# lambdaclass/simpleworks

Hardware: AMD Instinct MI355X
Metric: Marlin prove() constraints/sec at 2^20 R1CS; G1 MSM points/sec (higher is better)
Workload: dtype u32 limbs (384-bit Montgomery Fq for G1, 256-bit Fr); 1 GPU; marlin_prove: synthetic R1CS, 2^20 constraints = variables = non-zeros per matrix (|H| = |K| = 2^20), SRS + proving key device resident; per_gpu_units=1048576, multi_gpu=replicas (one proof per rank)

## Files before the change

### simpleworks_amd/_lib.py

```python
import ctypes
import json
import os

import numpy as np

_HERE = os.path.dirname(os.path.abspath(__file__))
LIB_PATH = os.environ.get("SWM_LIB_PATH") or os.path.join(_HERE, "libswmarlin.so")

_u64p = ctypes.POINTER(ctypes.c_uint64)
_u32p = ctypes.POINTER(ctypes.c_uint32)
_vp = ctypes.c_void_p
_sz = ctypes.c_size_t
_int = ctypes.c_int

ABI = {
    "swm_version": (_int, []),
    "swm_strerror": (ctypes.c_char_p, [_int]),
    "swm_init": (_int, [_int, ctypes.POINTER(_vp)]),
    "swm_destroy": (None, [_vp]),
    "swm_last_error": (ctypes.c_char_p, [_vp]),
    "swm_set_stream": (_int, [_vp, _vp]),
    "swm_set_msm_sharding": (_int, [_vp, ctypes.c_uint, ctypes.c_uint, _vp, _vp]),
    "swm_rccl_unique_id": (_int, [ctypes.c_void_p]),
    "swm_rccl_init": (_int, [_vp, ctypes.c_void_p, ctypes.c_uint, ctypes.c_uint]),
# ... 971 lines not shown
                                              _p64(out), _p64(jac) if backmap else None, _p32(status), n), "swm_selftest_p28")
        return out, status[:n], jac

    def _poly(self, op, data, n, m, z, pieces, out):
        zz = np.ascontiguousarray(z if z is not None else np.zeros(4), dtype=np.uint64).reshape(4)
        pc = np.ascontiguousarray(pieces if pieces is not None else np.zeros(2), dtype=np.uint64).reshape(-1)
        self._check(self.lib.swm_selftest_poly(self.h, op, data.ctypes.data, n, m, _p64(zz), _p64(pc), pc.size // 2,
                                               out.ctypes.data if out is not None else None), "swm_selftest_poly")

    def selftest_suffix_recurrence(self, a_mont, m, z_mont):
        a = np.ascontiguousarray(a_mont, dtype=np.uint64).reshape(-1, 4).copy()
        self._poly(0, a, a.shape[0], m, z_mont, None, None)
        return a

    def selftest_div_linear(self, p_mont, z_mont):
        p = np.ascontiguousarray(p_mont, dtype=np.uint64).reshape(-1, 4)
        out = np.zeros_like(p)
        self._poly(1, p, p.shape[0], 0, z_mont, None, out)
        return out

    def selftest_poly_eval(self, p_mont, z_mont):
        p = np.ascontiguousarray(p_mont, dtype=np.uint64).reshape(-1, 4)
        out = np.zeros(4, dtype=np.uint64)
        self._poly(2, p, p.shape[0], 0, z_mont, None, out)
        return out

    def selftest_poly_eval_many(self, buf_mont, pieces, z_mont):
        buf = np.ascontiguousarray(buf_mont, dtype=np.uint64).reshape(-1, 4)
        pc = np.asarray(pieces, dtype=np.uint64).reshape(-1, 2)
        out = np.zeros((pc.shape[0], 4), dtype=np.uint64)
        self._poly(3, buf, buf.shape[0], 0, z_mont, pc, out)
        return out

    def selftest_ntt_from(self, src_mont, log_n, inverse=False, coset=False):
        src = np.ascontiguousarray(src_mont, dtype=np.uint64).reshape(-1, 4).copy()
        out = np.zeros((1 << log_n, 4), dtype=np.uint64)
        self._poly(4 + int(bool(inverse)) + 2 * int(bool(coset)), src, src.shape[0], log_n, None, None, out)
        return out, src

    def selftest_ntt_cosets(self, coeffs_mont, log_n, ks):
        src = np.ascontiguousarray(coeffs_mont, dtype=np.uint64).reshape(-1, 4).copy()
        kk = np.ascontiguousarray(ks, dtype=np.uint64).reshape(-1)
        out = np.zeros((kk.size << log_n, 4), dtype=np.uint64)
        self._check(self.lib.swm_selftest_poly(self.h, 9, src.ctypes.data, src.shape[0], log_n, _p64(np.zeros(4, np.uint64)),
                                               _p64(kk), kk.size, out.ctypes.data), "swm_selftest_poly")
        return out.reshape(kk.size, 1 << log_n, 4)

    def selftest_intt_cosets3(self, evals_mont, log_n):
        ev = np.ascontiguousarray(evals_mont, dtype=np.uint64).reshape(-1, 4).copy()
        out = np.zeros_like(ev)
        self._poly(10, ev, ev.shape[0], log_n, None, None, out)
        return out

    def selftest_scan(self, words):
        w = np.ascontiguousarray(words, dtype=np.uint32).reshape(-1)
        out = np.zeros(w.size + 1, dtype=np.uint32)
        self._poly(8, w, w.size, 0, None, None, out)
        return out[:-1], int(out[-1])

    def selftest_sample_fr(self, rng, need):
        out = np.zeros((max(need, 1), 4), dtype=np.uint64)
        self._check(self.lib.swm_selftest_sample_fr(self.h, rng.h, need, _p64(out)), "swm_selftest_sample_fr")
        return out[:need]

    def selftest_mul_throughput(self, which, threads, iters):
        ms = ctypes.c_float(0)
        self._check(self.lib.swm_selftest_mul_throughput(self.h, which, threads, iters, ctypes.byref(ms)),
                    "swm_selftest_mul_throughput")
        return ms.value
```

### simpleworks_amd/csrc/fr29.cuh

```cuda
#pragma once
#include "ff.cuh"

namespace swm {

struct Fr29 {
    uint32_t l[9];
};
static constexpr uint32_t M29 = (1u << 29) - 1;
struct Fr29Consts {
    static constexpr uint32_t P[9] = SWM_FR29_P;
    static constexpr uint32_t ONE[9] = SWM_FR29_ONE;
    static constexpr uint32_t P2[9] = SWM_FR29_2P;
};

__device__ __forceinline__ Fr29 fr29_unpack(const Fr& a) {
    Fr29 r;
#pragma unroll
    for (int i = 0; i < 9; i++) {
        const int bit = 29 * i, w = bit >> 5, off = bit & 31;
        uint32_t v = a.v[w] >> off;
        if (off > 3 && w + 1 < 8) v |= a.v[w + 1] << (32 - off);
        r.l[i] = i < 8 ? (v & M29) : v;
    }
    return r;
}
__device__ __forceinline__ Fr fr29_pack(const Fr29& a) {
    Fr r;
#pragma unroll
    for (int w = 0; w < 8; w++) {
        const int bit = 32 * w, i = bit / 29, off = bit - 29 * i;
        uint32_t v = a.l[i] >> off;
        if (i + 1 < 9) v |= a.l[i + 1] << (29 - off);
        if (29 - off + 29 < 32 && i + 2 < 9) v |= a.l[i + 2] << (58 - off);
        r.v[w] = v;
    }
    return r;
}
__device__ __forceinline__ Fr29 fr29_const(const uint32_t (&c)[9]) {
    Fr29 r;
#pragma unroll
    for (int i = 0; i < 9; i++) r.l[i] = c[i];
    return r;
}
__device__ __forceinline__ Fr29 fr29_normalize(const Fr29& a) {
    Fr29 r;
    uint32_t c = 0;
#pragma unroll
    for (int i = 0; i < 8; i++) {
        uint32_t t = a.l[i] + c;
        r.l[i] = t & M29;
        c = t >> 29;
    }
    r.l[8] = a.l[8] + c;
    return r;
}
__device__ __forceinline__ Fr29 fr29_add(const Fr29& a, const Fr29& b) {
    Fr29 r;
#pragma unroll
    for (int i = 0; i < 9; i++) r.l[i] = a.l[i] + b.l[i];
    return r;
}
struct Spread29 {
    uint32_t l[9];
};
__device__ __forceinline__ Fr29 fr29_sub(const Fr29& a, const Fr29& b, const Spread29& sp) {
    Fr29 r;
#pragma unroll
    for (int i = 0; i < 9; i++) r.l[i] = a.l[i] + sp.l[i] - b.l[i];
    return r;
}
__device__ __forceinline__ Fr29 fr29_mul(const Fr29& a, const Fr29& b) {
    Fr29 r;
    uint32_t m[9];
    uint64_t acc = 0;
#pragma unroll
    for (int k = 0; k < 9; k++) {
#pragma unroll
        for (int i = 0; i <= k; i++) acc += (uint64_t)a.l[i] * b.l[k - i];
#pragma unroll
        for (int i = 0; i < k; i++) acc += (uint64_t)m[i] * Fr29Consts::P[k - i];
        m[k] = (0u - (uint32_t)acc) & M29;
        acc = (acc + m[k]) >> 29;
    }
#pragma unroll
    for (int k = 9; k < 17; k++) {
#pragma unroll
        for (int i = k - 8; i < 9; i++) acc += (uint64_t)a.l[i] * b.l[k - i];
#pragma unroll
        for (int i = k - 8; i < 9; i++) acc += (uint64_t)m[i] * Fr29Consts::P[k - i];
        r.l[k - 9] = (uint32_t)acc & M29;
        acc >>= 29;
    }
    r.l[8] = (uint32_t)acc;
    return r;
}
#include "fr29_mul_asm.inc"
__device__ __forceinline__ Fr29 fr29_mul_fenced(const Fr29& a, const Fr29& b) {
    Fr29 r;
    uint32_t m0, m1, m2, m3, m4, m5, m6, m7, m8;
    constexpr const uint32_t (&P)[9] = Fr29Consts::P;
    static_assert(P[0] == 1u, "the carry rule needs r = 1 mod 2^29");
    asm(SWM_FR29_MUL_ASM_TEXT
        : "=&v"(r.l[0]), "=&v"(r.l[1]), "=&v"(r.l[2]), "=&v"(r.l[3]), "=&v"(r.l[4]), "=&v"(r.l[5]), "=&v"(r.l[6]), "=&v"(r.l[7]),
          "=&v"(r.l[8]), "=&v"(m0), "=&v"(m1), "=&v"(m2), "=&v"(m3), "=&v"(m4), "=&v"(m5), "=&v"(m6), "=&v"(m7), "=&v"(m8)
        : "v"(a.l[0]), "v"(a.l[1]), "v"(a.l[2]), "v"(a.l[3]), "v"(a.l[4]), "v"(a.l[5]), "v"(a.l[6]), "v"(a.l[7]), "v"(a.l[8]),
          "v"(b.l[0]), "v"(b.l[1]), "v"(b.l[2]), "v"(b.l[3]), "v"(b.l[4]), "v"(b.l[5]), "v"(b.l[6]), "v"(b.l[7]), "v"(b.l[8]),
          "s"(P[1]), "s"(P[2]), "s"(P[3]), "s"(P[4]), "s"(P[5]), "s"(P[6]), "s"(P[7]), "s"(P[8]), "s"(M29), "s"((uint64_t)M29)
        : "v0", "v1", "vcc");
    return r;
}
__device__ __forceinline__ Fr29 fr29_cond_sub(const Fr29& a, const uint32_t (&k)[9]) {
    Fr29 t;
    uint32_t borrow = 0;
#pragma unroll
    for (int i = 0; i < 9; i++) {
        uint32_t d = a.l[i] - k[i] - borrow;
        borrow = d >> 31;
        t.l[i] = i < 8 ? (d & M29) : d;
    }
    Fr29 r;
#pragma unroll
// ... 10 lines not shown
```

### simpleworks_amd/csrc/marlin.hip

```cpp
#include <stdlib.h>
#include <string.h>
#include <algorithm>
#include <chrono>
#include <functional>
#include <memory>
#include <type_traits>
#include "devops.cuh"
#include "g1.cuh"
#include "host/ahp.h"

#include "msm.h"
using namespace swm;

#define LAUNCHX(ctx, name, kernel, grid, block, shmem, ...)                         \
    do {                                                                            \
        prof_begin(ctx, name);                                                      \
        hipLaunchKernelGGL(kernel, grid, block, shmem, (ctx)->stream, __VA_ARGS__); \
        prof_end(ctx);                                                              \
        hip_check(ctx, hipGetLastError(), name);                                    \
    } while (0)

#include "host/pk_codec.h"
#include "host/host_handles.h"
struct swm_srs {
// ... 2330 lines not shown
    SWM_ON_DEVICE(ctx);
    SWM_GUARD(ctx, *out = pk_deserialize(ctx, bytes, len, (flags & SWM_KEY_UNCOMPRESSED) != 0, !(flags & SWM_KEY_UNCHECKED)));
}
int swm_pk_deserialize(swm_ctx* ctx, const uint8_t* bytes, size_t len, swm_pk** out) {
    return swm_pk_deserialize_ex(ctx, bytes, len, 0, out);
}
int swm_r1cs_is_satisfied(swm_ctx* ctx, const swm_r1cs* cs, int* ok, size_t* first_bad) {
    if (!ctx || !cs || !ok) return SWM_ERR_INVALID_ARG;
    SWM_ON_DEVICE(ctx);
    SWM_GUARD(ctx, is_satisfied_impl(ctx, cs, ok, first_bad));
}

static void selftest_poly_impl(swm_ctx* ctx, int op, void* data, size_t n, size_t m, const uint64_t* z, const uint64_t* pieces,
                               size_t npieces, void* out) {
    Fr zz = fp_zero<Fr>();
    if (z) memcpy(zz.v, z, 32);
    if (op == 8) {
        DBuf<uint32_t> in(ctx, n), res(ctx, n);
        if (n) in.upload((const uint32_t*)data, n);
        const uint32_t total = scan_exclusive_u32(ctx, in.p, res.p, n);
        std::vector<uint32_t> h = res.download(0, n);
        if (n) memcpy(out, h.data(), n * 4);
        ((uint32_t*)out)[n] = total;
        return;
    }
    DVec a(ctx, n);
    if (n) a.upload((const Fr*)data, n);
    if (op == 9) {
        unsigned ks[4];
        for (size_t c = 0; c < npieces; c++) ks[c] = (unsigned)pieces[c];
        DVec t(ctx, npieces << m);
        rc_check(ctx, ntt_cosets_fwd(ctx, a.p, n, (unsigned)m, ks, (unsigned)npieces, t.p));
        std::vector<Fr> h = t.download(0, t.n);
        memcpy(out, h.data(), t.n * sizeof(Fr));
        return;
    }
    if (op == 10) {
        const size_t N = (size_t)1 << m;
        rc_check(ctx, ntt_cosets_inv(ctx, a.p, (unsigned)m, 3));
        DVec t(ctx, 3 * N);
        const Fr* u = a.p;
        Fr* o = t.p;
        const Fr iota = HDomain(4).gen, half = fr_half();
        ew(ctx, "cosets3_solve", N, [=] __device__(size_t j) {
            const Cosets3 c = cosets3_solve(u[j], u[j + N], u[j + 2 * N], iota, half);
            o[j] = c.p0;
            o[j + N] = c.p1;
            o[j + 2 * N] = c.p2;
        });
        std::vector<Fr> h = t.download(0, t.n);
        memcpy(out, h.data(), t.n * sizeof(Fr));
        return;
    }
    if (op == 0) {
        suffix_recurrence(ctx, a.p, n, m, zz);
        std::vector<Fr> h = a.download(0, n);
        if (n) memcpy(data, h.data(), n * sizeof(Fr));
    } else if (op == 1) {
        DivResult r = div_linear(ctx, a.p, n, zz);
        std::vector<Fr> h = r.work.download(0, n);
        if (n) memcpy(out, h.data(), n * sizeof(Fr));
    } else if (op == 2) {
        const Fr v = poly_eval(ctx, a.p, n, zz);
        memcpy(out, v.v, sizeof(Fr));
    } else if (op == 3) {
        for (size_t i = 0; i < npieces; i++)
            if (pieces[2 * i] > n || pieces[2 * i + 1] > n - pieces[2 * i]) throw MarlinError(SWM_ERR_INVALID_ARG, "piece out of range");
        DVec res(ctx, npieces);
        std::vector<EvalItem> items;
        for (size_t i = 0; i < npieces; i++) items.push_back({a.p + pieces[2 * i], (size_t)pieces[2 * i + 1], res.p + i});
        EvalPoint ep = eval_point(ctx, zz);
        poly_eval_many(ctx, items, ep);
        std::vector<Fr> h = res.download(0, npieces);
        if (npieces) memcpy(out, h.data(), npieces * sizeof(Fr));
    } else {
        DVec t = dv_ntt_from(ctx, a.p, n, (unsigned)m, ((op - 4) & 1) != 0, ((op - 4) & 2) != 0);
        std::vector<Fr> h = t.download(0, t.n);
        memcpy(out, h.data(), t.n * sizeof(Fr));
        std::vector<Fr> s = a.download(0, n);
        if (n) memcpy(data, s.data(), n * sizeof(Fr));
    }
}
int swm_selftest_poly(swm_ctx* ctx, int op, void* data, size_t n, size_t m, const uint64_t z[4], const uint64_t* pieces,
                      size_t npieces, void* out) {
    if (!ctx || op < 0 || op > 10 || (n && !data)) return SWM_ERR_INVALID_ARG;
    if ((op >= 1 && op <= 3 && !z) || (op == 0 && (!z || m == 0)) || (op != 0 && !out) || (op == 3 && npieces && !pieces))
        return SWM_ERR_INVALID_ARG;
    if (op >= 4 && op <= 7 && (m < 1 || m > 28 || n > ((size_t)1 << m))) return SWM_ERR_INVALID_ARG;
    if (op == 9) {
        if (m < 1 || m > 26 || n > ((size_t)2 << m) || npieces < 1 || npieces > 4 || !pieces) return SWM_ERR_INVALID_ARG;
        for (size_t c = 0; c < npieces; c++)
            if (pieces[c] > 3) return SWM_ERR_INVALID_ARG;
    }
    if (op == 10 && (m < 1 || m > 26 || n != ((size_t)3 << m))) return SWM_ERR_INVALID_ARG;
    SWM_ON_DEVICE(ctx);
    SWM_GUARD(ctx, selftest_poly_impl(ctx, op, data, n, m, z, pieces, npieces, out));
}
static void selftest_sample_impl(swm_ctx* ctx, ChaChaRng& rng, size_t need, uint64_t* out_mont) {
    DVec d(ctx, need);
    sample_fr_bulk(ctx, rng, d.p, need);
    std::vector<Fr> h = d.download(0, need);
    if (need) memcpy(out_mont, h.data(), need * sizeof(Fr));
}
int swm_selftest_sample_fr(swm_ctx* ctx, swm_rng* rng, size_t need, uint64_t* out_mont) {
    if (!ctx || !rng || (need && !out_mont)) return SWM_ERR_INVALID_ARG;
    SWM_ON_DEVICE(ctx);
    SWM_GUARD(ctx, selftest_sample_impl(ctx, rng->r, need, out_mont));
}

static void selftest_g1_codec_impl(swm_ctx* ctx, int op, const void* in, size_t n, void* out, unsigned* bad) {
    const dim3 grid((unsigned)((n + 255) / 256)), block(256);
    if (op == 0) {
        DBuf<G1Affine> pts(ctx, n);
        DBuf<uint32_t> enc(ctx, n * 24);
        pts.upload((const G1Affine*)in, n);
        LAUNCHX(ctx, "g1_encode_uncompressed", g1_encode_uncompressed_kernel, grid, block, 0, pts.p, n, enc.p);
        std::vector<uint32_t> h = enc.download(0, n * 24);
        memcpy(out, h.data(), n * 96);
        return;
    }
    DBuf<uint32_t> enc(ctx, n * 24), flag(ctx, 1);
    DBuf<G1Affine> pts(ctx, n);
    flag.zero();
    enc.upload((const uint32_t*)in, n * 24);
    if (op == 1) LAUNCHX(ctx, "g1_decode_uncompressed", g1_decode_uncompressed_kernel<true>, grid, block, 0, enc.p, n, pts.p, flag.p);
    else LAUNCHX(ctx, "g1_decode_unchecked", g1_decode_uncompressed_kernel<false>, grid, block, 0, enc.p, n, pts.p, flag.p);
    *bad = flag.download(0, 1)[0];
    std::vector<G1Affine> h = pts.download(0, n);
    memcpy(out, h.data(), n * sizeof(G1Affine));
}
int swm_selftest_g1_codec(swm_ctx* ctx, int op, const void* in, size_t n, void* out, unsigned* bad) {
    if (!ctx || op < 0 || op > 2 || (n && (!in || !out)) || (op != 0 && !bad) || n > ((size_t)1 << 31)) return SWM_ERR_INVALID_ARG;
    SWM_ON_DEVICE(ctx);
    if (op != 0) *bad = 0;
    if (n == 0) return SWM_OK;
    SWM_GUARD(ctx, selftest_g1_codec_impl(ctx, op, in, n, out, bad));
}

// ... 41 lines not shown
```

### simpleworks_amd/csrc/ntt.hip

```cpp
#include <atomic>
#include "context.h"
#include "ff.cuh"
#include "fr29.cuh"
#include <string.h>
#include <algorithm>
#include <vector>

namespace swm {

static constexpr int NTT_THREADS = 256;
static constexpr unsigned NTT_MAX_LOG_R = 10;

struct NttPassArgs {
    const Fr* src;
    Fr* dst;
    unsigned log_n, log_r, log_ns;
    const Fr* tw_small;
    const Fr* tw_lo;
    const Fr* tw_hi;
    const Fr* cs_lo;
    const Fr* cs_hi;
    uint64_t src_len;
    const Fr* pass_tw;
    int coset_in;
// ... 73 lines not shown
    for (; h >= 2; h >>= 2) {
        const unsigned hh = h >> 1, s1 = (R >> 1) / h, s2 = 2 * s1;
        for (unsigned q = threadIdx.x; q < (R >> 2) * J; q += NTT_THREADS) {
            unsigned jj = q % J, qq = q / J;
            unsigned p = qq & (hh - 1), blk = qq / hh;
            unsigned i0 = blk * 2 * h + p, i1 = i0 + hh, i2 = i0 + h, i3 = i2 + hh;
            Fr x0 = tile[i0 * J + jj], x1 = tile[i1 * J + jj], x2 = tile[i2 * J + jj], x3 = tile[i3 * J + jj];
            Fr a0 = fp_add(x0, x2), a2 = fp_sub(x0, x2);
            if (p) a2 = fp_mul(a2, a.tw_small[p * s1]);
            Fr a1 = fp_add(x1, x3), a3 = fp_mul(fp_sub(x1, x3), a.tw_small[(p + hh) * s1]);
            Fr y1 = fp_sub(a0, a1), y3 = fp_sub(a2, a3);
            if (p) {
                Fr w = a.tw_small[p * s2];
                y1 = fp_mul(y1, w);
                y3 = fp_mul(y3, w);
            }
            tile[i0 * J + jj] = fp_add(a0, a1);
            tile[i1 * J + jj] = y1;
            tile[i2 * J + jj] = fp_add(a2, a3);
            tile[i3 * J + jj] = y3;
        }
        __syncthreads();
    }
    for (unsigned e = threadIdx.x; e < R * J; e += NTT_THREADS) {
        unsigned jj, u;
        if (a.log_ns == 0) {
            u = e % R;
            jj = e / R;
        } else {
            jj = e % J;
            u = e / J;
        }
        uint64_t j = j0 + jj;
        uint64_t k = j & ns_mask;
        uint64_t o = ((j - k) << a.log_r) + k + ((uint64_t)u << a.log_ns);
        Fr x = tile[bitrev_u(u, a.log_r) * J + jj];
        if (a.scale_out) {
            Fr s = a.n_inv;
            if (a.coset_out) s = fp_mul(s, two_level_pow(a.cs_lo, a.cs_hi, o * cs_k));
            x = fp_mul(x, s);
        }
        dst[o] = x;
    }
}

struct LazyPlan {
    Spread29 r2;
    Spread29 s1[6];
    Spread29 s2[6];
    Spread29 s4;
    uint32_t reduce;
    uint32_t out_below_2r;
};
struct NttLazyArgs {
    NttPassArgs a;
    LazyPlan plan;
    int last_pass;
};
__device__ __forceinline__ Fr29 two_level_pow29(const Fr* lo, const Fr* hi, uint64_t e) {
    Fr29 a = fr29_unpack(lo[e & 1023]);
    uint64_t h = e >> 10;
    if (h) a = fr29_mul_fenced(a, fr29_unpack(hi[h]));
    return a;
}
__device__ __forceinline__ unsigned tile_slot(unsigned idx) { return (idx + (idx >> 5)) * 9; }
__device__ __forceinline__ void tile_put(uint32_t* tile, unsigned idx, const Fr29& x) {
    const unsigned o = tile_slot(idx);
#pragma unroll
    for (int i = 0; i < 9; i++) tile[o + i] = x.l[i];
}
__device__ __forceinline__ Fr29 tile_get(const uint32_t* tile, unsigned idx) {
    const unsigned o = tile_slot(idx);
    Fr29 x;
#pragma unroll
    for (int i = 0; i < 9; i++) x.l[i] = tile[o + i];
    return x;
}
template <int J>
__global__ void __launch_bounds__(NTT_THREADS, 4) ntt_pass_lazy(NttLazyArgs args) {
    SWM_LIGHT_KERNEL();
    extern __shared__ __align__(16) unsigned char smem_raw[];
    uint32_t* tile = reinterpret_cast<uint32_t*>(smem_raw);
    const NttPassArgs& a = args.a;
    const LazyPlan& P = args.plan;
    const unsigned R = 1u << a.log_r;
    const uint64_t n = 1ull << a.log_n;
    const uint64_t stride = n >> a.log_r;
    const uint64_t j0 = (uint64_t)blockIdx.x * J;
    const uint64_t ns_mask = (1ull << a.log_ns) - 1;
    const unsigned tw_shift = a.log_n - a.log_ns - a.log_r;
    const Fr* src = a.src + blockIdx.y * a.src_cstride;
    Fr* dst = a.dst + blockIdx.y * a.dst_cstride;
    const uint64_t cs_k = a.cos_k[blockIdx.y];
    for (unsigned e0 = 0; e0 < R * J; e0 += 4 * NTT_THREADS) {
        Fr xs[4];
#pragma unroll
        for (int u = 0; u < 4; u++) {
            unsigned e = e0 + threadIdx.x + u * NTT_THREADS;
            if (e < R * J) {
                const uint64_t at = j0 + e % J + (uint64_t)(e / J) * stride;
                xs[u] = at < a.src_len ? src[at] : fp_zero<Fr>();
                if (a.fold_in && at + n < a.src_len) xs[u] = fp_add(xs[u], fp_mul(a.fold[blockIdx.y], src[at + n]));
            }
        }
#pragma unroll
        for (int u = 0; u < 4; u++) {
            unsigned e = e0 + threadIdx.x + u * NTT_THREADS;
            if (e >= R * J) break;
            unsigned jj = e % J, t = e / J;
            uint64_t idx = j0 + jj + (uint64_t)t * stride;
            Fr29 x = fr29_unpack(xs[u]);
            if (a.coset_in) x = fr29_mul_fenced(x, two_level_pow29(a.cs_lo, a.cs_hi, idx * cs_k));
            if (a.log_ns != 0) {
                uint64_t k = (j0 + jj) & ns_mask;
                const Fr29 tw = a.pass_tw ? fr29_unpack(a.pass_tw[((uint64_t)t << a.log_ns) + k])
                                          : two_level_pow29(a.tw_lo, a.tw_hi, (k * t) << tw_shift);
                x = fr29_mul_fenced(x, tw);
            }
            tile_put(tile, t * J + jj, x);
        }
    }
    __syncthreads();
    unsigned h = R >> 1;
    if (a.log_r & 1) {
        for (unsigned bq = threadIdx.x; bq < (R >> 1) * J; bq += NTT_THREADS) {
            unsigned jj = bq % J, pos = bq / J;
            unsigned i0 = pos, i1 = i0 + h;
            Fr29 u = tile_get(tile, i0 * J + jj), v = tile_get(tile, i1 * J + jj);
            tile_put(tile, i0 * J + jj, fr29_normalize(fr29_add(u, v)));
            tile_put(tile, i1 * J + jj, fr29_mul_fenced(fr29_sub(u, v, P.r2), fr29_unpack(a.tw_small[pos])));
        }
        h >>= 1;
        __syncthreads();
    }
    unsigned step = 0;
    for (; h >= 2; h >>= 2, step++) {
        const unsigned hh = h >> 1, s1 = (R >> 1) / h, s2 = 2 * s1;
        const bool red = (P.reduce >> step) & 1u;
        const Spread29& S1 = P.s1[step];
        const Spread29& S2 = P.s2[step];
        for (unsigned q = threadIdx.x; q < (R >> 2) * J; q += NTT_THREADS) {
            unsigned jj = q % J, qq = q / J;
            unsigned p = qq & (hh - 1), blk = qq / hh;
            unsigned i0 = blk * 2 * h + p, i1 = i0 + hh, i2 = i0 + h, i3 = i2 + hh;
            Fr29 a0, a1, a2, a3;
            {
                Fr29 x0 = tile_get(tile, i0 * J + jj), x2 = tile_get(tile, i2 * J + jj);
                a0 = fr29_add(x0, x2);
                a2 = fr29_mul_fenced(fr29_sub(x0, x2, S1), fr29_unpack(a.tw_small[p * s1]));
            }
            {
                Fr29 x1 = tile_get(tile, i1 * J + jj), x3 = tile_get(tile, i3 * J + jj);
                a1 = fr29_add(x1, x3);
                a3 = fr29_mul_fenced(fr29_sub(x1, x3, S1), fr29_unpack(a.tw_small[(p + hh) * s1]));
            }
            const Fr29 w = fr29_unpack(a.tw_small[p * s2]);
            Fr29 y0 = fr29_add(a0, a1);
            y0 = red ? fr29_mul_fenced(y0, fr29_const(Fr29Consts::ONE)) : fr29_normalize(y0);
            tile_put(tile, i0 * J + jj, y0);
            tile_put(tile, i1 * J + jj, fr29_mul_fenced(fr29_sub(a0, a1, S2), w));
            tile_put(tile, i2 * J + jj, fr29_normalize(fr29_add(a2, a3)));
            tile_put(tile, i3 * J + jj, fr29_mul_fenced(fr29_sub(a2, a3, P.s4), w));
        }
        __syncthreads();
    }
    for (unsigned e = threadIdx.x; e < R * J; e += NTT_THREADS) {
        unsigned jj, u;
        if (a.log_ns == 0) {
            u = e % R;
            jj = e / R;
        } else {
            jj = e % J;
            u = e / J;
        }
        uint64_t j = j0 + jj;
        uint64_t k = j & ns_mask;
        uint64_t o = ((j - k) << a.log_r) + k + ((uint64_t)u << a.log_ns);
        Fr29 x = tile_get(tile, bitrev_u(u, a.log_r) * J + jj);
        if (a.scale_out) {
            Fr29 sc = fr29_unpack(a.n_inv);
            if (a.coset_out) sc = fr29_mul_fenced(two_level_pow29(a.cs_lo, a.cs_hi, o * cs_k), sc);
            x = fr29_canonical(fr29_mul_fenced(x, sc), true);
        } else if (args.last_pass) {
            x = fr29_canonical(x, P.out_below_2r != 0);
        }
        dst[o] = fr29_pack(x);
    }
}

static Fr host_root_of_unity(unsigned log_n, bool inverse) {
    Fr w;
    const uint32_t root[8] = SWM_FR_ROOT47_MONT;
    for (int i = 0; i < 8; i++) w.v[i] = root[i];
    for (unsigned i = log_n; i < 47; i++) w = fp_sqr(w);
    if (inverse) w = fp_inv(w);
    return w;
}

static int upload_powers(swm_ctx* ctx, const Fr& base, size_t count, void** out, bool lazy29 = false) {
    std::vector<Fr> h(count);
    Fr cur = lazy29 ? fp_from_u64<Fr>(32) : fp_one<Fr>();
    for (size_t i = 0; i < count; i++) {
        h[i] = cur;
        cur = fp_mul(cur, base);
    }
    SWM_HIP(ctx, hipMalloc(out, count * sizeof(Fr)));
    SWM_HIP(ctx, hipMemcpy(*out, h.data(), count * sizeof(Fr), hipMemcpyHostToDevice));
    return SWM_OK;
}

static int two_level_tables(swm_ctx* ctx, const Fr& base, size_t max_exp, NttTables* t, bool lazy29 = false) {
    SWM_TRY(upload_powers(ctx, base, 1024, &t->lo, lazy29));
    Fr b1024 = base;
    for (int i = 0; i < 10; i++) b1024 = fp_sqr(b1024);
    t->hi_len = (max_exp >> 10) + 1;
    SWM_TRY(upload_powers(ctx, b1024, t->hi_len, &t->hi, lazy29));
    return SWM_OK;
}
static constexpr uint64_t LAZY_KEY = 1ull << 50;

static int get_root_tables_form(swm_ctx* ctx, unsigned log_n, int inverse, bool lazy29, NttTables** out) {
    uint64_t key = ((uint64_t)log_n << 1) | (inverse ? 1 : 0) | (lazy29 ? LAZY_KEY : 0);
    auto it = ctx->ntt_tables.find(key);
    if (it == ctx->ntt_tables.end()) {
        NttTables t;
        SWM_TRY(two_level_tables(ctx, host_root_of_unity(log_n, inverse), 1ull << log_n, &t, lazy29));
        it = ctx->ntt_tables.emplace(key, t).first;
    }
    *out = &it->second;
    return SWM_OK;
}

int get_root_tables(swm_ctx* ctx, unsigned log_n, int inverse, NttTables** out) {
    return get_root_tables_form(ctx, log_n, inverse, false, out);
}

static int get_coset_tables(swm_ctx* ctx, unsigned log_n, int inverse, NttTables** out, bool lazy29 = false) {
    uint64_t key = (1ull << 40) | (inverse ? 1 : 0) | (lazy29 ? LAZY_KEY : 0);
    auto it = ctx->ntt_tables.find(key);
    if (it != ctx->ntt_tables.end() && it->second.hi_len < ((1ull << log_n) >> 10) + 1) {
        (void)hipFree(it->second.lo);
        (void)hipFree(it->second.hi);
        ctx->ntt_tables.erase(it);
        it = ctx->ntt_tables.end();
    }
    if (it == ctx->ntt_tables.end()) {
        Fr g;
        const uint32_t gm[8] = SWM_FR_GEN_MONT, gi[8] = SWM_FR_GEN_INV_MONT;
        for (int i = 0; i < 8; i++) g.v[i] = inverse ? gi[i] : gm[i];
        NttTables t;
        unsigned cap = log_n < 20 ? 20 : log_n;
        SWM_TRY(two_level_tables(ctx, g, 1ull << cap, &t, lazy29));
        it = ctx->ntt_tables.emplace(key, t).first;
    }
    *out = &it->second;
    return SWM_OK;
}

static int get_small_table(swm_ctx* ctx, unsigned log_r, int inverse, const Fr** out, bool lazy29 = false) {
    uint64_t key = ((uint64_t)log_r << 1) | (inverse ? 1 : 0) | (lazy29 ? LAZY_KEY : 0);
    auto it = ctx->ntt_small.find(key);
    if (it == ctx->ntt_small.end()) {
        void* d = nullptr;
        size_t cnt = log_r ? (1u << (log_r - 1)) : 1;
        SWM_TRY(upload_powers(ctx, host_root_of_unity(log_r, inverse), cnt, &d, lazy29));
        it = ctx->ntt_small.emplace(key, d).first;
    }
    *out = reinterpret_cast<const Fr*>(it->second);
    return SWM_OK;
}

__global__ void __launch_bounds__(256) ntt_build_pass_tw(const Fr* __restrict__ lo29, const Fr* __restrict__ hi29, unsigned log_ns,
                                                         unsigned log_r, unsigned shift, Fr* __restrict__ out) {
    const uint64_t x = blockIdx.x * (uint64_t)blockDim.x + threadIdx.x;
    if (x >> (log_ns + log_r)) return;
    const uint64_t k = x & (((uint64_t)1 << log_ns) - 1), t = x >> log_ns;
    out[x] = fr29_pack(fr29_canonical(two_level_pow29(lo29, hi29, (k * t) << shift), true));
}
static int get_pass_table(swm_ctx* ctx, unsigned log_n, int inverse, unsigned log_ns, unsigned log_r, const NttTables* rt29,
                          const Fr** out) {
    *out = nullptr;
    static const bool off = sw(SW_NTT_PASS_TABLES) == 0;
    if (off) return SWM_OK;
    const uint64_t key = (1ull << 51) | ((uint64_t)log_n << 20) | ((uint64_t)log_ns << 10) | ((uint64_t)log_r << 1) | (inverse ? 1 : 0);
    auto it = ctx->ntt_small.find(key);
    if (it == ctx->ntt_small.end()) {
        const size_t count = (size_t)1 << (log_ns + log_r);
        if (ctx->ntt_pass_table_bytes + count * sizeof(Fr) > ((size_t)4 << 30)) return SWM_OK;
        void* d = nullptr;
        if (hipMalloc(&d, count * sizeof(Fr)) != hipSuccess) {
            (void)hipGetLastError();
            return SWM_OK;
        }
        hipLaunchKernelGGL(ntt_build_pass_tw, dim3((unsigned)((count + 255) / 256)), dim3(256), 0, ctx->stream,
                           reinterpret_cast<const Fr*>(rt29->lo), reinterpret_cast<const Fr*>(rt29->hi), log_ns, log_r,
                           log_n - log_ns - log_r, reinterpret_cast<Fr*>(d));
        SWM_HIP(ctx, hipGetLastError());
        ctx->ntt_pass_table_bytes += count * sizeof(Fr);
        it = ctx->ntt_small.emplace(key, d).first;
    }
    *out = reinterpret_cast<const Fr*>(it->second);
    return SWM_OK;
}

static Spread29 lazy_spread(unsigned k, unsigned borrows) {
    Spread29 sp;
    uint64_t carry = 0;
    for (int i = 0; i < 9; i++) {
        uint64_t t = (uint64_t)Fr29Consts::P[i] * k + carry;
        sp.l[i] = i < 8 ? (uint32_t)(t & M29) : (uint32_t)t;
        carry = t >> 29;
    }
    sp.l[0] += borrows << 29;
    for (int i = 1; i < 8; i++) sp.l[i] += (borrows << 29) - borrows;
    sp.l[8] -= borrows;
    return sp;
}
static LazyPlan lazy_plan(unsigned log_r, unsigned b_in) {
    LazyPlan P;
    memset(&P, 0, sizeof(P));
    unsigned B = b_in;
    P.r2 = lazy_spread(2 * B, 1);
    if (log_r & 1) B = std::max(2 * B, 2u);
    const unsigned nsteps = log_r / 2;
    for (unsigned st = 0; st < nsteps && st < 6; st++) {
        P.s1[st] = lazy_spread(2 * B, 1);
        P.s2[st] = lazy_spread(4 * B, 2);
        const bool red = 4 * B > 64 || st + 1 == nsteps;
        if (red) P.reduce |= 1u << st;
        B = red ? 4 : 4 * B;
    }
    P.s4 = lazy_spread(4, 1);
    P.out_below_2r = B <= 2 ? 1u : 0u;
    return P;
}

int ntt_run_from(swm_ctx* ctx, void* d_data, unsigned log_n, int inverse, int coset, const void* first_src, size_t src_len);
int ntt_run(swm_ctx* ctx, void* d_data, unsigned log_n, int inverse, int coset) {
    return ntt_run_from(ctx, d_data, log_n, inverse, coset, nullptr, 0);
}
static int ntt_run_multi(swm_ctx* ctx, void* d_data, unsigned log_n, int inverse, int coset, const void* first_src, size_t src_len,
                         unsigned ncos, const unsigned* ks);
int ntt_run_from(swm_ctx* ctx, void* d_data, unsigned log_n, int inverse, int coset, const void* first_src, size_t src_len) {
    if (first_src && src_len > (1ull << std::min(log_n, 62u))) src_len = 1ull << log_n;
    return ntt_run_multi(ctx, d_data, log_n, inverse, coset ? 1 : 0, first_src, src_len, 1, nullptr);
}
int ntt_cosets_fwd(swm_ctx* ctx, const void* coeffs, size_t len, unsigned log_n, const unsigned* ks, unsigned ncos, void* out) {
    if (ncos < 1 || ncos > 4 || log_n > 28 || len > (2ull << log_n)) return set_err(ctx, SWM_ERR_INVALID_ARG, "ntt cosets: bad shape");
    for (unsigned c = 0; c < ncos; c++)
        if (ks[c] > 3) return set_err(ctx, SWM_ERR_INVALID_ARG, "ntt cosets: coset index > 3");
    return ntt_run_multi(ctx, out, log_n, 0, 2, coeffs, len, ncos, ks);
}
int ntt_cosets_inv(swm_ctx* ctx, void* data, unsigned log_n, unsigned ncos) {
    if (ncos < 1 || ncos > 4 || log_n > 28) return set_err(ctx, SWM_ERR_INVALID_ARG, "ntt cosets: bad shape");
    const unsigned ks[4] = {0, 1, 2, 3};
    return ntt_run_multi(ctx, data, log_n, 1, 2, nullptr, 0, ncos, ks);
}
static int ntt_run_multi(swm_ctx* ctx, void* d_data, unsigned log_n, int inverse, int coset, const void* first_src, size_t src_len,
                         unsigned ncos, const unsigned* ks) {
    if (log_n > 30) return set_err(ctx, SWM_ERR_INVALID_ARG, "ntt: log_n > 30 unsupported");
    const uint64_t n = 1ull << log_n;
    for (unsigned c = 0; c < ncos; c++) {
        ctx->stat_ntt_calls++;
        ctx->log_call('n', log_n);
        ctx->stat_ntt_elems += n;
    }
    Fr* data = reinterpret_cast<Fr*>(d_data);
    const uint64_t total = n * ncos;
    const unsigned maxr = NTT_MAX_LOG_R;
    static const bool lazy = sw(SW_NTT_LAZY) != 0;
    NttTables *rt = nullptr, *ct = nullptr;
    SWM_TRY(get_root_tables_form(ctx, log_n, inverse, lazy, &rt));
    if (coset == 1) SWM_TRY(get_coset_tables(ctx, log_n, inverse, &ct, lazy));
    if (coset == 2) SWM_TRY(get_root_tables_form(ctx, log_n + 2, inverse, lazy, &ct));
    Fr fold[4];
    for (unsigned c = 0; c < 4; c++) {
        fold[c] = fp_one<Fr>();
        if (coset == 2 && c < ncos)
            for (unsigned e = 0; e < ks[c]; e++) fold[c] = fp_mul(fold[c], host_root_of_unity(2, false));
    }
    Fr n_inv = fp_one<Fr>();
    if (inverse) n_inv = fp_inv(fp_from_u64<Fr>(n));
    if (lazy) n_inv = fp_mul(n_inv, fp_from_u64<Fr>(32));
    unsigned npass = log_n <= maxr ? 1 : (log_n + maxr - 1) / maxr;
    unsigned radices[8];
    {
        unsigned rem = log_n;
        for (unsigned p = 0; p < npass; p++) {
            unsigned r = (rem + (npass - p) - 1) / (npass - p);
            radices[p] = r;
            rem -= r;
        }
    }
    Fr *tmp = nullptr, *tmp2 = nullptr;
    SWM_TRY(scratch(ctx, "ntt.tmp", total * sizeof(Fr), (void**)&tmp));
    if (npass % 2 == 1 && npass >= 3) SWM_TRY(scratch(ctx, "ntt.tmp2", total * sizeof(Fr), (void**)&tmp2));
    const Fr* src = first_src ? reinterpret_cast<const Fr*>(first_src) : data;
    if (npass == 1 && !first_src) {
        SWM_HIP(ctx, hipMemcpyAsync(tmp, data, total * sizeof(Fr), hipMemcpyDeviceToDevice, ctx->stream));
        src = tmp;
    }
    unsigned log_ns = 0;
    for (unsigned p = 0; p < npass; p++) {
        NttPassArgs a;
        a.src = src;
        if (p == npass - 1) a.dst = data;
        else if (tmp2) a.dst = (p % 2 == 0) ? tmp : tmp2;
        else a.dst = (src == tmp) ? data : tmp;
        a.src_len = (p == 0 && first_src) ? (uint64_t)src_len : n;
        a.log_n = log_n;
        a.log_r = radices[p];
        a.log_ns = log_ns;
        SWM_TRY(get_small_table(ctx, a.log_r, inverse, &a.tw_small, lazy));
        a.tw_lo = reinterpret_cast<const Fr*>(rt->lo);
        a.tw_hi = reinterpret_cast<const Fr*>(rt->hi);
        a.cs_lo = ct ? reinterpret_cast<const Fr*>(ct->lo) : nullptr;
        a.cs_hi = ct ? reinterpret_cast<const Fr*>(ct->hi) : nullptr;
        a.pass_tw = nullptr;
        if (lazy && log_ns != 0) SWM_TRY(get_pass_table(ctx, log_n, inverse, log_ns, a.log_r, rt, &a.pass_tw));
        a.coset_in = (coset && !inverse && p == 0) ? 1 : 0;
        a.scale_out = (inverse && p == npass - 1) ? 1 : 0;
        a.coset_out = (coset && inverse && p == npass - 1) ? 1 : 0;
        a.n_inv = n_inv;
        a.src_cstride = (p == 0 && first_src) ? 0 : n;
        a.dst_cstride = n;
        a.fold_in = (coset == 2 && a.coset_in && src_len > n) ? 1 : 0;
        for (unsigned c = 0; c < 4; c++) {
            a.cos_k[c] = coset == 2 ? (c < ncos ? ks[c] : 0) : 1;
            a.fold[c] = fold[c];
        }
        uint64_t cols = n >> a.log_r;
        if (lazy) {
            NttLazyArgs la;
            la.a = a;
            la.plan = lazy_plan(a.log_r, (p > 0 || a.coset_in) ? 2u : 1u);
            la.last_pass = p == npass - 1 ? 1 : 0;
            unsigned J = 1;
            if (npass > 1) {
                J = (log_n >= 19 ? 1024u : 512u) >> a.log_r;
                if (J < 1) J = 1;
                if (J > 16) J = 16;
                while (J > cols) J >>= 1;
            }
            const size_t elems = (size_t)J << a.log_r;
            size_t shmem = (elems + (elems >> 5) + 1) * 36;
            if (shmem < 64) shmem = 64;
            dim3 grid((unsigned)(cols / J), ncos), block(NTT_THREADS);
            if (shmem > 64 * 1024) {
                static std::atomic<size_t> granted[64];
                if (J != 1 || shmem > 160 * 1024) return set_err(ctx, SWM_ERR_INVALID_ARG, "ntt: tile does not fit LDS");
                if (granted[ctx->device & 63].load() < shmem) {
                    SWM_HIP(ctx, hipFuncSetAttribute((const void*)ntt_pass_lazy<1>, hipFuncAttributeMaxDynamicSharedMemorySize, (int)shmem));
                    granted[ctx->device & 63].store(shmem);
                }
            }
            switch (J) {
                case 1: SWM_LAUNCH(ctx, "ntt_pass", ntt_pass_lazy<1>, grid, block, shmem, la); break;
                case 2: SWM_LAUNCH(ctx, "ntt_pass", ntt_pass_lazy<2>, grid, block, shmem, la); break;
                case 4: SWM_LAUNCH(ctx, "ntt_pass", ntt_pass_lazy<4>, grid, block, shmem, la); break;
                case 8: SWM_LAUNCH(ctx, "ntt_pass", ntt_pass_lazy<8>, grid, block, shmem, la); break;
                default: SWM_LAUNCH(ctx, "ntt_pass", ntt_pass_lazy<16>, grid, block, shmem, la); break;
            }
        } else if (npass == 1) {
            size_t shmem = sizeof(Fr) << a.log_r;
            if (shmem < 64) shmem = 64;
            SWM_LAUNCH(ctx, "ntt_pass", ntt_pass<1>, dim3((unsigned)cols, ncos), dim3(NTT_THREADS), shmem, a);
        } else {
            unsigned J = (log_n >= 19 ? 1024u : 512u) >> a.log_r;
            if (J < 1) J = 1;
            if (J > 16) J = 16;
            while (J > cols) J >>= 1;
            size_t shmem = (sizeof(Fr) * J) << a.log_r;
            dim3 grid((unsigned)(cols / J), ncos), block(NTT_THREADS);
            switch (J) {
                case 1: SWM_LAUNCH(ctx, "ntt_pass", ntt_pass<1>, grid, block, shmem, a); break;
                case 2: SWM_LAUNCH(ctx, "ntt_pass", ntt_pass<2>, grid, block, shmem, a); break;
                case 4: SWM_LAUNCH(ctx, "ntt_pass", ntt_pass<4>, grid, block, shmem, a); break;
                case 8: SWM_LAUNCH(ctx, "ntt_pass", ntt_pass<8>, grid, block, shmem, a); break;
                default: SWM_LAUNCH(ctx, "ntt_pass", ntt_pass<16>, grid, block, shmem, a); break;
            }
        }
        log_ns += a.log_r;
        src = a.dst;
    }
    return SWM_OK;
}


__global__ void __launch_bounds__(256) ntt_shard_twiddle(Fr* __restrict__ v, size_t count, const Fr* __restrict__ lo,
// ... 71 lines not shown
```

Baseline: 22.92 million constraints/s.

## Store lazy NTT twiddles in 29-bit limb form and fold inverse scaling into tables

Lazy-path twiddle, coset and pass tables are now stored pre-unpacked as Fr29 limbs, so the kernels no longer unpack each loaded twiddle. The inverse scaling by n^-1 is folded into the coset tables or into the last radix-4 step of the final pass, which drops a separate multiply at output. Reduction by multiplying with ONE is replaced by a quotient-estimate lazy reduction. Tables take 36 bytes per element instead of 32, so they use somewhat more memory bandwidth, and the scaled tables and new reduction carry correctness risk at the bounds. A selftest op for coset inverse NTT is also added.

```diff
diff --git a/simpleworks_amd/_lib.py b/simpleworks_amd/_lib.py
--- a/simpleworks_amd/_lib.py
+++ b/simpleworks_amd/_lib.py
@@ -1047,6 +1047,12 @@
         self._poly(10, ev, ev.shape[0], log_n, None, None, out)
         return out
 
+    def selftest_intt_cosets(self, evals_mont, log_n):
+        ev = np.ascontiguousarray(evals_mont, dtype=np.uint64).reshape(-1, 4).copy()
+        out = np.zeros_like(ev)
+        self._poly(11, ev, ev.shape[0], log_n, None, None, out)
+        return out.reshape(-1, 1 << log_n, 4)
+
     def selftest_scan(self, words):
         w = np.ascontiguousarray(words, dtype=np.uint32).reshape(-1)
         out = np.zeros(w.size + 1, dtype=np.uint32)
diff --git a/simpleworks_amd/csrc/fr29.cuh b/simpleworks_amd/csrc/fr29.cuh
--- a/simpleworks_amd/csrc/fr29.cuh
+++ b/simpleworks_amd/csrc/fr29.cuh
@@ -13,7 +13,7 @@
     static constexpr uint32_t P2[9] = SWM_FR29_2P;
 };
 
-__device__ __forceinline__ Fr29 fr29_unpack(const Fr& a) {
+__host__ __device__ __forceinline__ Fr29 fr29_unpack(const Fr& a) {
     Fr29 r;
 #pragma unroll
     for (int i = 0; i < 9; i++) {
@@ -67,6 +67,32 @@
     Fr29 r;
 #pragma unroll
     for (int i = 0; i < 9; i++) r.l[i] = a.l[i] + sp.l[i] - b.l[i];
+    return r;
+}
+__device__ __forceinline__ Fr29 fr29_reduce_lazy(const Fr29& a) {
+    constexpr const uint32_t (&P)[9] = Fr29Consts::P;
+    static_assert(P[0] == 1u, "limb 0 of q r is q");
+    constexpr uint32_t K = (uint32_t)((1ull << 52) / (P[8] + 1));
+    static_assert(((1ull << 52) / (P[8] + 1)) >> 32 == 0, "the reciprocal fits a word");
+    const uint32_t q = __umulhi(a.l[8], K) >> 20;
+    uint32_t qr[9];
+    qr[0] = q;
+    uint64_t c = 0;
+#pragma unroll
+    for (int i = 1; i < 9; i++) {
+        const uint64_t t = (uint64_t)q * P[i] + c;
+        qr[i] = i < 8 ? ((uint32_t)t & M29) : (uint32_t)t;
+        c = t >> 29;
+    }
+    Fr29 r;
+    uint32_t cy = 0;
+#pragma unroll
+    for (int i = 0; i < 8; i++) {
+        const uint32_t t = a.l[i] + (P[i] + (1u << 29) - (i ? 1u : 0u)) - qr[i] + cy;
+        r.l[i] = t & M29;
+        cy = t >> 29;
+    }
+    r.l[8] = a.l[8] + (P[8] - 1u) - qr[8] + cy;
     return r;
 }
 __device__ __forceinline__ Fr29 fr29_mul(const Fr29& a, const Fr29& b) {
diff --git a/simpleworks_amd/csrc/marlin.hip b/simpleworks_amd/csrc/marlin.hip
--- a/simpleworks_amd/csrc/marlin.hip
+++ b/simpleworks_amd/csrc/marlin.hip
@@ -2406,6 +2406,12 @@
         memcpy(out, h.data(), t.n * sizeof(Fr));
         return;
     }
+    if (op == 11) {
+        rc_check(ctx, ntt_cosets_inv(ctx, a.p, (unsigned)m, (unsigned)(n >> m)));
+        std::vector<Fr> h = a.download(0, n);
+        memcpy(out, h.data(), n * sizeof(Fr));
+        return;
+    }
     if (op == 0) {
         suffix_recurrence(ctx, a.p, n, m, zz);
         std::vector<Fr> h = a.download(0, n);
@@ -2437,7 +2443,8 @@
 }
 int swm_selftest_poly(swm_ctx* ctx, int op, void* data, size_t n, size_t m, const uint64_t z[4], const uint64_t* pieces,
                       size_t npieces, void* out) {
-    if (!ctx || op < 0 || op > 10 || (n && !data)) return SWM_ERR_INVALID_ARG;
+    if (!ctx || op < 0 || op > 11 || (n && !data)) return SWM_ERR_INVALID_ARG;
+    if (op == 11 && (m < 1 || m > 26 || (n >> m) < 1 || (n >> m) > 4 || n != ((n >> m) << m))) return SWM_ERR_INVALID_ARG;
     if ((op >= 1 && op <= 3 && !z) || (op == 0 && (!z || m == 0)) || (op != 0 && !out) || (op == 3 && npieces && !pieces))
         return SWM_ERR_INVALID_ARG;
     if (op >= 4 && op <= 7 && (m < 1 || m > 28 || n > ((size_t)1 << m))) return SWM_ERR_INVALID_ARG;
diff --git a/simpleworks_amd/csrc/ntt.hip b/simpleworks_amd/csrc/ntt.hip
--- a/simpleworks_amd/csrc/ntt.hip
+++ b/simpleworks_amd/csrc/ntt.hip
@@ -149,15 +149,24 @@
     uint32_t reduce;
     uint32_t out_below_2r;
 };
+struct LazyTables {
+    const Fr29* tw_small;
+    const Fr29 *tw_lo, *tw_hi;
+    const Fr29 *cs_lo, *cs_hi;
+    const Fr29* pass_tw;
+    const Fr29* fin;
+};
 struct NttLazyArgs {
     NttPassArgs a;
+    LazyTables t;
     LazyPlan plan;
     int last_pass;
+    int scale_step;
 };
-__device__ __forceinline__ Fr29 two_level_pow29(const Fr* lo, const Fr* hi, uint64_t e) {
-    Fr29 a = fr29_unpack(lo[e & 1023]);
+__device__ __forceinline__ Fr29 two_level_pow29(const Fr29* lo, const Fr29* hi, uint64_t e) {
+    Fr29 a = lo[e & 1023];
     uint64_t h = e >> 10;
-    if (h) a = fr29_mul_fenced(a, fr29_unpack(hi[h]));
+    if (h) a = fr29_mul_fenced(a, hi[h]);
     return a;
 }
 __device__ __forceinline__ unsigned tile_slot(unsigned idx) { return (idx + (idx >> 5)) * 9; }
@@ -179,6 +188,7 @@
     extern __shared__ __align__(16) unsigned char smem_raw[];
     uint32_t* tile = reinterpret_cast<uint32_t*>(smem_raw);
     const NttPassArgs& a = args.a;
+    const LazyTables& T = args.t;
     const LazyPlan& P = args.plan;
     const unsigned R = 1u << a.log_r;
     const uint64_t n = 1ull << a.log_n;
@@ -207,11 +217,11 @@
             unsigned jj = e % J, t = e / J;
             uint64_t idx = j0 + jj + (uint64_t)t * stride;
             Fr29 x = fr29_unpack(xs[u]);
-            if (a.coset_in) x = fr29_mul_fenced(x, two_level_pow29(a.cs_lo, a.cs_hi, idx * cs_k));
+            if (a.coset_in) x = fr29_mul_fenced(x, two_level_pow29(T.cs_lo, T.cs_hi, idx * cs_k));
             if (a.log_ns != 0) {
                 uint64_t k = (j0 + jj) & ns_mask;
-                const Fr29 tw = a.pass_tw ? fr29_unpack(a.pass_tw[((uint64_t)t << a.log_ns) + k])
-                                          : two_level_pow29(a.tw_lo, a.tw_hi, (k * t) << tw_shift);
+                const Fr29 tw = T.pass_tw ? T.pass_tw[((uint64_t)t << a.log_ns) + k]
+                                          : two_level_pow29(T.tw_lo, T.tw_hi, (k * t) << tw_shift);
                 x = fr29_mul_fenced(x, tw);
             }
             tile_put(tile, t * J + jj, x);
@@ -225,7 +235,7 @@
             unsigned i0 = pos, i1 = i0 + h;
             Fr29 u = tile_get(tile, i0 * J + jj), v = tile_get(tile, i1 * J + jj);
             tile_put(tile, i0 * J + jj, fr29_normalize(fr29_add(u, v)));
-            tile_put(tile, i1 * J + jj, fr29_mul_fenced(fr29_sub(u, v, P.r2), fr29_unpack(a.tw_small[pos])));
+            tile_put(tile, i1 * J + jj, fr29_mul_fenced(fr29_sub(u, v, P.r2), T.tw_small[pos]));
         }
         h >>= 1;
         __syncthreads();
@@ -236,28 +246,34 @@
         const bool red = (P.reduce >> step) & 1u;
         const Spread29& S1 = P.s1[step];
         const Spread29& S2 = P.s2[step];
+        const bool fin = (int)step == args.scale_step;
         for (unsigned q = threadIdx.x; q < (R >> 2) * J; q += NTT_THREADS) {
             unsigned jj = q % J, qq = q / J;
             unsigned p = qq & (hh - 1), blk = qq / hh;
             unsigned i0 = blk * 2 * h + p, i1 = i0 + hh, i2 = i0 + h, i3 = i2 + hh;
+            const Fr29 *wa = T.tw_small + p * s1, *wb = T.tw_small + (p + hh) * s1, *wc = T.tw_small + p * s2;
+            if (fin) wa = T.fin, wb = T.fin + 1, wc = T.fin;
             Fr29 a0, a1, a2, a3;
             {
                 Fr29 x0 = tile_get(tile, i0 * J + jj), x2 = tile_get(tile, i2 * J + jj);
                 a0 = fr29_add(x0, x2);
-                a2 = fr29_mul_fenced(fr29_sub(x0, x2, S1), fr29_unpack(a.tw_small[p * s1]));
+                a2 = fr29_mul_fenced(fr29_sub(x0, x2, S1), *wa);
             }
             {
                 Fr29 x1 = tile_get(tile, i1 * J + jj), x3 = tile_get(tile, i3 * J + jj);
                 a1 = fr29_add(x1, x3);
-                a3 = fr29_mul_fenced(fr29_sub(x1, x3, S1), fr29_unpack(a.tw_small[(p + hh) * s1]));
-            }
-            const Fr29 w = fr29_unpack(a.tw_small[p * s2]);
+                a3 = fr29_mul_fenced(fr29_sub(x1, x3, S1), *wb);
+            }
+            const Fr29 w = *wc;
+            Fr29 w3 = w;
+            if (fin) w3 = T.fin[2];
             Fr29 y0 = fr29_add(a0, a1);
-            y0 = red ? fr29_mul_fenced(y0, fr29_const(Fr29Consts::ONE)) : fr29_normalize(y0);
+            if (fin) y0 = fr29_mul_fenced(y0, w);
+            else y0 = red ? fr29_reduce_lazy(y0) : fr29_normalize(y0);
             tile_put(tile, i0 * J + jj, y0);
             tile_put(tile, i1 * J + jj, fr29_mul_fenced(fr29_sub(a0, a1, S2), w));
             tile_put(tile, i2 * J + jj, fr29_normalize(fr29_add(a2, a3)));
-            tile_put(tile, i3 * J + jj, fr29_mul_fenced(fr29_sub(a2, a3, P.s4), w));
+            tile_put(tile, i3 * J + jj, fr29_mul_fenced(fr29_sub(a2, a3, P.s4), w3));
         }
         __syncthreads();
     }
@@ -274,10 +290,10 @@
         uint64_t k = j & ns_mask;
         uint64_t o = ((j - k) << a.log_r) + k + ((uint64_t)u << a.log_ns);
         Fr29 x = tile_get(tile, bitrev_u(u, a.log_r) * J + jj);
-        if (a.scale_out) {
-            Fr29 sc = fr29_unpack(a.n_inv);
-            if (a.coset_out) sc = fr29_mul_fenced(two_level_pow29(a.cs_lo, a.cs_hi, o * cs_k), sc);
-            x = fr29_canonical(fr29_mul_fenced(x, sc), true);
+        if (a.coset_out) {
+            x = fr29_canonical(fr29_mul_fenced(x, two_level_pow29(T.cs_lo, T.cs_hi, o * cs_k)), true);
+        } else if (a.scale_out) {
+            x = fr29_canonical(fr29_mul_fenced(x, T.fin[0]), true);
         } else if (args.last_pass) {
             x = fr29_canonical(x, P.out_below_2r != 0);
         }
@@ -294,20 +310,28 @@
     return w;
 }
 
-static int upload_powers(swm_ctx* ctx, const Fr& base, size_t count, void** out, bool lazy29 = false) {
+static int upload_powers(swm_ctx* ctx, const Fr& base, size_t count, void** out, bool lazy29 = false, const Fr* first = nullptr) {
     std::vector<Fr> h(count);
     Fr cur = lazy29 ? fp_from_u64<Fr>(32) : fp_one<Fr>();
+    if (first) cur = fp_mul(cur, *first);
     for (size_t i = 0; i < count; i++) {
         h[i] = cur;
         cur = fp_mul(cur, base);
     }
+    if (lazy29) {
+        std::vector<Fr29> l(count);
+        for (size_t i = 0; i < count; i++) l[i] = fr29_unpack(h[i]);
+        SWM_HIP(ctx, hipMalloc(out, count * sizeof(Fr29)));
+        SWM_HIP(ctx, hipMemcpy(*out, l.data(), count * sizeof(Fr29), hipMemcpyHostToDevice));
+        return SWM_OK;
+    }
     SWM_HIP(ctx, hipMalloc(out, count * sizeof(Fr)));
     SWM_HIP(ctx, hipMemcpy(*out, h.data(), count * sizeof(Fr), hipMemcpyHostToDevice));
     return SWM_OK;
 }
 
-static int two_level_tables(swm_ctx* ctx, const Fr& base, size_t max_exp, NttTables* t, bool lazy29 = false) {
-    SWM_TRY(upload_powers(ctx, base, 1024, &t->lo, lazy29));
+static int two_level_tables(swm_ctx* ctx, const Fr& base, size_t max_exp, NttTables* t, bool lazy29 = false, const Fr* scale = nullptr) {
+    SWM_TRY(upload_powers(ctx, base, 1024, &t->lo, lazy29, scale));
     Fr b1024 = base;
     for (int i = 0; i < 10; i++) b1024 = fp_sqr(b1024);
     t->hi_len = (max_exp >> 10) + 1;
@@ -315,13 +339,16 @@
     return SWM_OK;
 }
 static constexpr uint64_t LAZY_KEY = 1ull << 50;
-
-static int get_root_tables_form(swm_ctx* ctx, unsigned log_n, int inverse, bool lazy29, NttTables** out) {
-    uint64_t key = ((uint64_t)log_n << 1) | (inverse ? 1 : 0) | (lazy29 ? LAZY_KEY : 0);
+static constexpr uint64_t SCALED_KEY = 1ull << 52;
+
+static int get_root_tables_form(swm_ctx* ctx, unsigned log_n, int inverse, bool lazy29, NttTables** out, bool scaled = false) {
+    uint64_t key = ((uint64_t)log_n << 1) | (inverse ? 1 : 0) | (lazy29 ? LAZY_KEY : 0) | (scaled ? SCALED_KEY : 0);
     auto it = ctx->ntt_tables.find(key);
     if (it == ctx->ntt_tables.end()) {
         NttTables t;
-        SWM_TRY(two_level_tables(ctx, host_root_of_unity(log_n, inverse), 1ull << log_n, &t, lazy29));
+        Fr sc = fp_one<Fr>();
+        if (scaled) sc = fp_inv(fp_from_u64<Fr>(1ull << (log_n - 2)));
+        SWM_TRY(two_level_tables(ctx, host_root_of_unity(log_n, inverse), 1ull << log_n, &t, lazy29, scaled ? &sc : nullptr));
         it = ctx->ntt_tables.emplace(key, t).first;
     }
     *out = &it->second;
@@ -330,6 +357,22 @@
 
 int get_root_tables(swm_ctx* ctx, unsigned log_n, int inverse, NttTables** out) {
     return get_root_tables_form(ctx, log_n, inverse, false, out);
+}
+
+static int get_scaled_coset_tables(swm_ctx* ctx, unsigned log_n, NttTables** out) {
+    uint64_t key = (1ull << 40) | 1 | LAZY_KEY | SCALED_KEY | ((uint64_t)log_n << 1);
+    auto it = ctx->ntt_tables.find(key);
+    if (it == ctx->ntt_tables.end()) {
+        Fr g;
+        const uint32_t gi[8] = SWM_FR_GEN_INV_MONT;
+        for (int i = 0; i < 8; i++) g.v[i] = gi[i];
+        const Fr sc = fp_inv(fp_from_u64<Fr>(1ull << log_n));
+        NttTables t;
+        SWM_TRY(two_level_tables(ctx, g, 1ull << log_n, &t, true, &sc));
+        it = ctx->ntt_tables.emplace(key, t).first;
+    }
+    *out = &it->second;
+    return SWM_OK;
 }
 
 static int get_coset_tables(swm_ctx* ctx, unsigned log_n, int inverse, NttTables** out, bool lazy29 = false) {
@@ -354,7 +397,7 @@
     return SWM_OK;
 }
 
-static int get_small_table(swm_ctx* ctx, unsigned log_r, int inverse, const Fr** out, bool lazy29 = false) {
+static int get_small_table(swm_ctx* ctx, unsigned log_r, int inverse, const void** out, bool lazy29 = false) {
     uint64_t key = ((uint64_t)log_r << 1) | (inverse ? 1 : 0) | (lazy29 ? LAZY_KEY : 0);
     auto it = ctx->ntt_small.find(key);
     if (it == ctx->ntt_small.end()) {
@@ -363,19 +406,34 @@
         SWM_TRY(upload_powers(ctx, host_root_of_unity(log_r, inverse), cnt, &d, lazy29));
         it = ctx->ntt_small.emplace(key, d).first;
     }
-    *out = reinterpret_cast<const Fr*>(it->second);
-    return SWM_OK;
-}
-
-__global__ void __launch_bounds__(256) ntt_build_pass_tw(const Fr* __restrict__ lo29, const Fr* __restrict__ hi29, unsigned log_ns,
-                                                         unsigned log_r, unsigned shift, Fr* __restrict__ out) {
+    *out = it->second;
+    return SWM_OK;
+}
+
+static int get_fin_table(swm_ctx* ctx, unsigned log_n, const Fr29** out) {
+    const uint64_t key = (1ull << 53) | ((uint64_t)log_n << 1) | 1;
+    auto it = ctx->ntt_small.find(key);
+    if (it == ctx->ntt_small.end()) {
+        const Fr to261 = fp_from_u64<Fr>(32), n_inv = fp_mul(fp_inv(fp_from_u64<Fr>(1ull << log_n)), to261);
+        const Fr29 h[3] = {fr29_unpack(n_inv), fr29_unpack(fp_mul(n_inv, host_root_of_unity(2, true))), fr29_unpack(to261)};
+        void* d = nullptr;
+        SWM_HIP(ctx, hipMalloc(&d, sizeof(h)));
+        SWM_HIP(ctx, hipMemcpy(d, h, sizeof(h), hipMemcpyHostToDevice));
+        it = ctx->ntt_small.emplace(key, d).first;
+    }
+    *out = reinterpret_cast<const Fr29*>(it->second);
+    return SWM_OK;
+}
+
+__global__ void __launch_bounds__(256) ntt_build_pass_tw(const Fr29* __restrict__ lo29, const Fr29* __restrict__ hi29, unsigned log_ns,
+                                                         unsigned log_r, unsigned shift, Fr29* __restrict__ out) {
     const uint64_t x = blockIdx.x * (uint64_t)blockDim.x + threadIdx.x;
     if (x >> (log_ns + log_r)) return;
     const uint64_t k = x & (((uint64_t)1 << log_ns) - 1), t = x >> log_ns;
-    out[x] = fr29_pack(fr29_canonical(two_level_pow29(lo29, hi29, (k * t) << shift), true));
+    out[x] = fr29_canonical(two_level_pow29(lo29, hi29, (k * t) << shift), true);
 }
 static int get_pass_table(swm_ctx* ctx, unsigned log_n, int inverse, unsigned log_ns, unsigned log_r, const NttTables* rt29,
-                          const Fr** out) {
+                          const Fr29** out) {
     *out = nullptr;
     static const bool off = sw(SW_NTT_PASS_TABLES) == 0;
     if (off) return SWM_OK;
@@ -383,20 +441,20 @@
     auto it = ctx->ntt_small.find(key);
     if (it == ctx->ntt_small.end()) {
         const size_t count = (size_t)1 << (log_ns + log_r);
-        if (ctx->ntt_pass_table_bytes + count * sizeof(Fr) > ((size_t)4 << 30)) return SWM_OK;
+        if (ctx->ntt_pass_table_bytes + count * sizeof(Fr29) > ((size_t)4 << 30)) return SWM_OK;
         void* d = nullptr;
-        if (hipMalloc(&d, count * sizeof(Fr)) != hipSuccess) {
+        if (hipMalloc(&d, count * sizeof(Fr29)) != hipSuccess) {
             (void)hipGetLastError();
             return SWM_OK;
         }
         hipLaunchKernelGGL(ntt_build_pass_tw, dim3((unsigned)((count + 255) / 256)), dim3(256), 0, ctx->stream,
-                           reinterpret_cast<const Fr*>(rt29->lo), reinterpret_cast<const Fr*>(rt29->hi), log_ns, log_r,
-                           log_n - log_ns - log_r, reinterpret_cast<Fr*>(d));
+                           reinterpret_cast<const Fr29*>(rt29->lo), reinterpret_cast<const Fr29*>(rt29->hi), log_ns, log_r,
+                           log_n - log_ns - log_r, reinterpret_cast<Fr29*>(d));
         SWM_HIP(ctx, hipGetLastError());
-        ctx->ntt_pass_table_bytes += count * sizeof(Fr);
+        ctx->ntt_pass_table_bytes += count * sizeof(Fr29);
         it = ctx->ntt_small.emplace(key, d).first;
     }
-    *out = reinterpret_cast<const Fr*>(it->second);
+    *out = reinterpret_cast<const Fr29*>(it->second);
     return SWM_OK;
 }
 
@@ -468,8 +526,9 @@
     static const bool lazy = sw(SW_NTT_LAZY) != 0;
     NttTables *rt = nullptr, *ct = nullptr;
     SWM_TRY(get_root_tables_form(ctx, log_n, inverse, lazy, &rt));
-    if (coset == 1) SWM_TRY(get_coset_tables(ctx, log_n, inverse, &ct, lazy));
-    if (coset == 2) SWM_TRY(get_root_tables_form(ctx, log_n + 2, inverse, lazy, &ct));
+    if (coset == 1 && lazy && inverse) SWM_TRY(get_scaled_coset_tables(ctx, log_n, &ct));
+    else if (coset == 1) SWM_TRY(get_coset_tables(ctx, log_n, inverse, &ct, lazy));
+    if (coset == 2) SWM_TRY(get_root_tables_form(ctx, log_n + 2, inverse, lazy, &ct, lazy && inverse));
     Fr fold[4];
     for (unsigned c = 0; c < 4; c++) {
         fold[c] = fp_one<Fr>();
@@ -478,7 +537,8 @@
     }
     Fr n_inv = fp_one<Fr>();
     if (inverse) n_inv = fp_inv(fp_from_u64<Fr>(n));
-    if (lazy) n_inv = fp_mul(n_inv, fp_from_u64<Fr>(32));
+    const Fr29* fin = nullptr;
+    if (lazy && inverse && !coset) SWM_TRY(get_fin_table(ctx, log_n, &fin));
     unsigned npass = log_n <= maxr ? 1 : (log_n + maxr - 1) / maxr;
     unsigned radices[8];
     {
@@ -508,13 +568,26 @@
         a.log_n = log_n;
         a.log_r = radices[p];
         a.log_ns = log_ns;
-        SWM_TRY(get_small_table(ctx, a.log_r, inverse, &a.tw_small, lazy));
-        a.tw_lo = reinterpret_cast<const Fr*>(rt->lo);
-        a.tw_hi = reinterpret_cast<const Fr*>(rt->hi);
-        a.cs_lo = ct ? reinterpret_cast<const Fr*>(ct->lo) : nullptr;
-        a.cs_hi = ct ? reinterpret_cast<const Fr*>(ct->hi) : nullptr;
-        a.pass_tw = nullptr;
-        if (lazy && log_ns != 0) SWM_TRY(get_pass_table(ctx, log_n, inverse, log_ns, a.log_r, rt, &a.pass_tw));
+        const void* small = nullptr;
+        SWM_TRY(get_small_table(ctx, a.log_r, inverse, &small, lazy));
+        a.tw_small = a.tw_lo = a.tw_hi = a.cs_lo = a.cs_hi = a.pass_tw = nullptr;
+        LazyTables lt;
+        memset(&lt, 0, sizeof(lt));
+        if (lazy) {
+            lt.tw_small = reinterpret_cast<const Fr29*>(small);
+            lt.tw_lo = reinterpret_cast<const Fr29*>(rt->lo);
+            lt.tw_hi = reinterpret_cast<const Fr29*>(rt->hi);
+            lt.cs_lo = ct ? reinterpret_cast<const Fr29*>(ct->lo) : nullptr;
+            lt.cs_hi = ct ? reinterpret_cast<const Fr29*>(ct->hi) : nullptr;
+            lt.fin = fin;
+            if (log_ns != 0) SWM_TRY(get_pass_table(ctx, log_n, inverse, log_ns, a.log_r, rt, &lt.pass_tw));
+        } else {
+            a.tw_small = reinterpret_cast<const Fr*>(small);
+            a.tw_lo = reinterpret_cast<const Fr*>(rt->lo);
+            a.tw_hi = reinterpret_cast<const Fr*>(rt->hi);
+            a.cs_lo = ct ? reinterpret_cast<const Fr*>(ct->lo) : nullptr;
+            a.cs_hi = ct ? reinterpret_cast<const Fr*>(ct->hi) : nullptr;
+        }
         a.coset_in = (coset && !inverse && p == 0) ? 1 : 0;
         a.scale_out = (inverse && p == npass - 1) ? 1 : 0;
         a.coset_out = (coset && inverse && p == npass - 1) ? 1 : 0;
@@ -530,8 +603,14 @@
         if (lazy) {
             NttLazyArgs la;
             la.a = a;
+            la.t = lt;
             la.plan = lazy_plan(a.log_r, (p > 0 || a.coset_in) ? 2u : 1u);
             la.last_pass = p == npass - 1 ? 1 : 0;
+            la.scale_step = -1;
+            if (a.scale_out && !a.coset_out && a.log_r >= 2) {
+                la.scale_step = (int)(a.log_r / 2) - 1;
+                la.a.scale_out = 0;
+            }
             unsigned J = 1;
             if (npass > 1) {
                 J = (log_n >= 19 ? 1024u : 512u) >> a.log_r;
```

Result: no change. 23.02 million constraints/s, median of 6 (+0.4%).
